# taekkii/deblurgs

Measured on AMD Instinct MI355X. Metric: subframe-renders/sec (fwd+bwd), 1M Gaussians, K=15, 1080p, 1/2/4/8 GPU, higher is better.
Workload: dtype f32; 1 GPU; metric: P=1000000 Gaussians, 1920x1080, K=15 subframes fused, curve_order=3, SH degree 2 (M=9); one blurry view per GPU per step; eager_preferred_steps=279, dropped_steps=0, retried_steps=0, tile_cull=True, depth_output=False, ranks_in_process_group=1

## Files before the change

### deblurgs_amd/build.py

```python
import glob
import hashlib
import json
import os
import subprocess
import sys
from concurrent.futures import ThreadPoolExecutor

HERE = os.path.dirname(os.path.abspath(__file__))
CSRC = os.path.join(HERE, "csrc")
OBJ = os.path.join(CSRC, "obj")
LIB = os.path.join(HERE, "libdgs_hip.so")
ARCH = "gfx950"
SOURCES = {
    "preprocess.hip": ["-ffp-contract=off"],
    "binning.hip": ["-ffp-contract=off"],
    "composite.hip": ["-fno-slp-vectorize"],
    "geometry_bwd.hip": [],
    "pose.hip": [],
    "knn.hip": [],
    "optim.hip": ["-ffp-contract=off"],
    "api.hip": [],
    "loss.hip": [],
    "metrics.hip": ["-ffp-contract=off"],
    "frames.hip": ["-ffp-contract=off"],
    "report.hip": ["-ffp-contract=off"],
    "lpips.hip": ["-ffp-contract=off"],
    "listprof.hip": [],
    "register.hip": [],
    "scene.hip": ["-ffp-contract=off"],
    "png.hip": [],
}
COMMON = ["-O3", "-fPIC", "-std=c++17", f"--offload-arch={ARCH}", "-fhip-fp32-correctly-rounded-divide-sqrt",
          "-Wall", "-Wno-unused-function"]


def _hipcc():
    for c in (os.environ.get("HIPCC"), "/opt/rocm/bin/hipcc", "hipcc"):
        if c and (os.path.isabs(c) and os.path.exists(c) or not os.path.isabs(c)):
            return c
    return "hipcc"


def _stale(target, deps):
    if not os.path.exists(target):
        return True
    t = os.path.getmtime(target)
    return any(os.path.getmtime(d) > t for d in deps)


HEADER = os.path.join(HERE, "..", "include", "dgs_hip.h")


def _sha(*chunks):
    h = hashlib.sha256()
    for c in chunks:
        h.update(c if isinstance(c, bytes) else c.encode())
        h.update(b"\0")
    return h.hexdigest()


def _read(path):
    with open(path, "rb") as f:
        return f.read()


def flag_table():
    return json.dumps({"common": COMMON, "sources": SOURCES, "arch": ARCH}, sort_keys=True)


def build_id(csrc=CSRC, header=HEADER):
    parts = []
    for f in sorted(glob.glob(os.path.join(csrc, "*.hip")) + glob.glob(os.path.join(csrc, "*.h"))):
        parts += [os.path.basename(f), _read(f)]
    parts += ["dgs_hip.h", _read(header), flag_table()]
    return _sha(*parts)


def _object_stamp(src, extra, headers, bid):
    return _sha(_read(src), *[_read(h) for h in headers], json.dumps(COMMON + extra), bid if src.endswith("api.hip") else "")


def _stamp_matches(path, want):
    try:
        with open(path) as f:
            return f.read().strip() == want
    except OSError:
        return False


SAN_LIB = os.path.join(HERE, "libdgs_hip_san.so")
SAN_OBJ = os.path.join(CSRC, "obj_san")
SAN_FLAGS = ["-O1", "-g", "-fno-omit-frame-pointer", "-fsanitize=address,undefined", "-fno-gpu-sanitize", "-shared-libsan",
             "-fno-sanitize-recover=undefined"]


def asan_runtime():
    r = subprocess.run([_hipcc(), "-print-file-name=libclang_rt.asan-x86_64.so"], capture_output=True, text=True)
    path = r.stdout.strip()
    if os.path.isabs(path) and os.path.exists(path):
        return path
    import glob
    hits = glob.glob("/opt/rocm/lib/llvm/lib/clang/*/lib/linux/libclang_rt.asan-x86_64.so")
    return hits[0] if hits else None


def build_sanitized(force=False, verbose=False):
    os.makedirs(SAN_OBJ, exist_ok=True)
    headers = [os.path.join(CSRC, "dgs_common.h"), os.path.join(HERE, "..", "include", "dgs_hip.h")]
    hipcc = _hipcc()
    common = [f for f in COMMON if f != "-O3"] + SAN_FLAGS
    jobs, objs = [], []
    for src, extra in SOURCES.items():
        s = os.path.join(CSRC, src)
        o = os.path.join(SAN_OBJ, src.replace(".hip", ".o"))
        objs.append(o)
        if force or _stale(o, [s] + headers):
            define = [f'-DDGS_BUILD_ID="{build_id()}"'] if src == "api.hip" else []
            jobs.append([hipcc] + common + extra + define + ["-c", s, "-o", o])

    def run(cmd):
        if verbose:
            print(" ".join(cmd), flush=True)
        r = subprocess.run(cmd, capture_output=True, text=True)
        if r.returncode != 0:
            raise RuntimeError("hipcc failed:\n" + " ".join(cmd) + "\n" + r.stdout + r.stderr)
        return r

    with ThreadPoolExecutor(max_workers=4) as ex:
        list(ex.map(run, jobs))
    if force or jobs or _stale(SAN_LIB, objs):
        run([hipcc, "-shared", "-fPIC", f"--offload-arch={ARCH}", "-fsanitize=address,undefined", "-shared-libsan",
             "-o", SAN_LIB] + objs)
    return SAN_LIB


def build(force=False, verbose=False):
    os.makedirs(OBJ, exist_ok=True)
    headers = [os.path.join(CSRC, "dgs_common.h"), HEADER]
    hipcc = _hipcc()
    bid = build_id()
    jobs = []
    objs = []
    stamps = []
    for src, extra in SOURCES.items():
        s = os.path.join(CSRC, src)
        o = os.path.join(OBJ, src.replace(".hip", ".o"))
        objs.append(o)
        want = _object_stamp(s, extra, headers, bid)
        if force or not os.path.exists(o) or not _stamp_matches(o + ".stamp", want):
            define = [f'-DDGS_BUILD_ID="{bid}"'] if src == "api.hip" else []
            jobs.append([hipcc] + COMMON + extra + define + ["-c", s, "-o", o])
            stamps.append((o + ".stamp", want))

    def run(cmd):
        if verbose:
            print(" ".join(cmd), flush=True)
        r = subprocess.run(cmd, capture_output=True, text=True)
        if r.returncode != 0:
            raise RuntimeError("hipcc failed:\n" + " ".join(cmd) + "\n" + r.stdout + r.stderr)
        return r

    with ThreadPoolExecutor(max_workers=4) as ex:
        list(ex.map(run, jobs))
    for path, want in stamps:
        with open(path, "w") as f:
            f.write(want + "\n")
    if force or jobs or not os.path.exists(LIB) or not _stamp_matches(LIB + ".stamp", bid):
        run([hipcc, "-shared", "-fPIC", f"--offload-arch={ARCH}", "-o", LIB] + objs)
        with open(LIB + ".stamp", "w") as f:
            f.write(bid + "\n")
    return LIB


if __name__ == "__main__":
    if "--sanitize" in sys.argv:
        print(build_sanitized(force="--force" in sys.argv, verbose=True))
    else:
        print(build(force="--force" in sys.argv, verbose=True))
```

### deblurgs_amd/csrc/api.hip

```cpp
#include <stdio.h>
#include <string.h>

#include <mutex>
#include <new>

#include "dgs_common.h"

namespace {

thread_local char g_err[512] = "";

int fail(int code, const char* fmt, const char* a = "") {
  snprintf(g_err, sizeof(g_err), fmt, a);
  return code;
}
int fail_hip(hipError_t e, const char* where) {
  snprintf(g_err, sizeof(g_err), "%s: %s", where, hipGetErrorString(e));
  return DGS_E_HIP;
}

constexpr size_t ALIGN = 256;
size_t up(size_t x) { return (x + ALIGN - 1) / ALIGN * ALIGN; }

int sort_bits_for(int W, int H, int K) {
// ... 53 lines not shown

int check_problem(const DgsProblem* p, bool need_opacity = true) {
  if (p == nullptr) return fail(DGS_E_ARG, "null DgsProblem");
  if (p->P < 0 || p->W <= 0 || p->H <= 0) return fail(DGS_E_ARG, "bad P/W/H");
  if (p->W > 4095 * DGS_TILE || p->H > 4095 * DGS_TILE) return fail(DGS_E_ARG, "W / H above 65520 pixels");
  if (p->K < 1 || p->K > DGS_MAX_K) return fail(DGS_E_ARG, "K must be in [1, DGS_MAX_K]");
  if (p->D < 0 || p->D > 3) return fail(DGS_E_ARG, "SH degree must be 0..3");
  if (p->forward_only != 0 && p->forward_only != 1) return fail(DGS_E_ARG, "forward_only must be 0 or 1");
  if (p->P == 0) return DGS_OK;
  if (p->means3D == nullptr || (need_opacity && p->opacities == nullptr))
    return fail(DGS_E_ARG, "means3D / opacities are null");
  if ((p->shs == nullptr) == (p->colors_precomp == nullptr))
    return fail(DGS_E_ARG, "Please provide excatly one of either SHs or precomputed colors!");
  if (((p->scales == nullptr || p->rotations == nullptr) && p->cov3D_precomp == nullptr) ||
      ((p->scales != nullptr || p->rotations != nullptr) && p->cov3D_precomp != nullptr))
    return fail(DGS_E_ARG, "Please provide exactly one of either scale/rotation pair or precomputed 3D covariance!");
  if (p->shs != nullptr && p->M < (p->D + 1) * (p->D + 1)) return fail(DGS_E_ARG, "M < (D+1)^2");
  if (p->raw_params != 0 && p->raw_params != 1 && p->raw_params != 3)
    return fail(DGS_E_ARG, "raw_params must be 0, 1 or 3 (1 | isotropic scale)");
  if (p->raw_params) {
    if (p->shs == nullptr || p->scales == nullptr || p->rotations == nullptr)
      return fail(DGS_E_ARG, "raw_params needs shs (dc), scales and rotations");
    if (p->M > 1 && p->shs_rest == nullptr) return fail(DGS_E_ARG, "raw_params with M > 1 needs shs_rest");
  } else if (p->shs_rest != nullptr) {
    return fail(DGS_E_ARG, "shs_rest is only meaningful with raw_params");
  }
  if (p->viewmatrix == nullptr || p->projmatrix == nullptr || p->campos == nullptr || p->bg == nullptr)
    return fail(DGS_E_ARG, "viewmatrix / projmatrix / campos / bg are null");
  if ((uint64_t)p->K * (uint64_t)p->P >= (1ull << 32)) return fail(DGS_E_ARG, "K*P must be < 2^32");
  return DGS_OK;
}

DgsView make_view(const DgsProblem* p, const DgsLayout& L) {
  DgsView v;
  v.P = p->P; v.D = p->D; v.M = p->M; v.W = p->W; v.H = p->H; v.K = p->K;
  v.gx = (p->W + DGS_TILE - 1) / DGS_TILE;
  v.gy = (p->H + DGS_TILE - 1) / DGS_TILE;
  v.T = v.gx * v.gy;
  v.tanfovx = p->tanfovx; v.tanfovy = p->tanfovy;
  v.focal_y = p->H / (2.0f * p->tanfovy);
  v.focal_x = p->W / (2.0f * p->tanfovx);
  v.scale_modifier = p->scale_modifier;
  v.z_far = p->z_far;
  v.use_sigmoid = p->use_sigmoid; v.prefiltered = p->prefiltered;
  v.tile_cull = p->tile_cull != 0;
  v.raw_params = (p->raw_params & 1) != 0;
  v.iso_scale = (p->raw_params & 2) != 0;
  v.pack_g_shift = v.tile_cull ? L.pack_g_shift : 0;
  v.pack_tile_shift = v.tile_cull ? L.pack_tile_shift : 0;
  v.scale_lb = p->scale_lb;
  return v;
}

void carve(const DgsProblem* p, const DgsLayout& L, DgsCarve* c) {
  char* g = reinterpret_cast<char*>(p->geom_state);
  char* im = reinterpret_cast<char*>(p->image_state);
  char* b = reinterpret_cast<char*>(p->binning_state);
  c->rows = reinterpret_cast<DgsRow*>(g + L.geom_rows);
  c->cov3D = p->forward_only ? nullptr : reinterpret_cast<float*>(g + L.cov3D);
  c->pre_sigmoid = p->forward_only ? nullptr : reinterpret_cast<float*>(g + L.pre_sigmoid);
  c->tiles_touched = reinterpret_cast<uint32_t*>(g + L.tiles_touched);
  c->point_offsets = reinterpret_cast<uint32_t*>(g + L.point_offsets);
  c->scan_tmp = reinterpret_cast<uint32_t*>(g + L.scan_tmp);
  c->num_rendered = reinterpret_cast<uint32_t*>(g + L.num_rendered);
  c->gsort_keys = reinterpret_cast<uint32_t*>(g + L.gsort_keys);
  c->gsort_keys_alt = reinterpret_cast<uint32_t*>(g + L.gsort_keys_alt);
  c->gsort_vals = reinterpret_cast<uint32_t*>(g + L.gsort_vals);
  c->gsort_vals_alt = reinterpret_cast<uint32_t*>(g + L.gsort_vals_alt);
  c->tt_sorted = reinterpret_cast<uint32_t*>(g + L.tt_sorted);
  c->offs_sorted = reinterpret_cast<uint32_t*>(g + L.offs_sorted);
  c->tt_tight = reinterpret_cast<uint32_t*>(g + L.tt_tight);
  c->offs_tight = reinterpret_cast<uint32_t*>(g + L.offs_tight);
  c->gsort_tmp = reinterpret_cast<uint32_t*>(g + L.gsort_tmp);
  c->cull_rec = reinterpret_cast<uint4*>(g + L.cull_rec);
  c->cull_cnt = reinterpret_cast<uint32_t*>(g + L.cull_cnt);
  c->final_T = p->forward_only ? nullptr : reinterpret_cast<float*>(im + L.final_T);
  c->n_contrib = p->forward_only ? nullptr : reinterpret_cast<uint32_t*>(im + L.n_contrib);
  c->ranges = reinterpret_cast<uint2*>(im + L.ranges);
  c->keys_sorted = b ? reinterpret_cast<uint64_t*>(b + L.keys_sorted) : nullptr;
  c->point_list = b ? reinterpret_cast<uint32_t*>(b + L.point_list) : nullptr;
  c->keys_unsorted = b ? reinterpret_cast<uint64_t*>(b + L.keys_unsorted) : nullptr;
  c->vals_unsorted = b ? reinterpret_cast<uint32_t*>(b + L.vals_unsorted) : nullptr;
  c->sort_tmp = b ? reinterpret_cast<uint32_t*>(b + L.sort_tmp) : nullptr;
}

struct ScratchLayout {
  size_t sums, partials, total;
};
ScratchLayout scratch_layout(uint64_t R, int P, int K) {
  const size_t sums = up((size_t)R * DGS_CONTRIB_F * 4);
  const size_t partials = sums + up((size_t)K * (size_t)P * DGS_SUMS_F * 4);
  return {sums, partials, partials + up((size_t)dgs_geometry_bwd_blocks(P) * (size_t)K * 24 * 8) + ALIGN};
}

struct Call {
  DgsLayout L;
  DgsCarve c;
  DgsView v;
  float* contrib = nullptr;
  float* sums = nullptr;
  double* partials = nullptr;
};
enum { NEED_IMAGE = 1, NEED_BINNING = 2 };
int prepare(const DgsProblem* p, uint64_t R, int need, const DgsBackwardIO* io, Call* k) {
  k->L = make_layout(p->P, p->W, p->H, p->K, R, p->wide_records != 0, p->forward_only != 0);
  if (p->geom_state == nullptr || p->geom_bytes < k->L.geom_total) return fail(DGS_E_CAPACITY, "geom_state too small");
  if ((need & NEED_IMAGE) && (p->image_state == nullptr || p->image_bytes < k->L.image_total))
    return fail(DGS_E_CAPACITY, "image_state too small");
  if ((need & NEED_BINNING) && R > 0 && (p->binning_state == nullptr || p->binning_bytes < k->L.binning_total))
    return fail(DGS_E_CAPACITY, "binning_state too small");
  carve(p, k->L, &k->c);
  k->v = make_view(p, k->L);
  if (io != nullptr) {
    const ScratchLayout sl = scratch_layout(R, p->P, p->K);
    if (io->scratch == nullptr || io->scratch_bytes < sl.total) return fail(DGS_E_CAPACITY, "backward scratch too small");
    char* base = reinterpret_cast<char*>(io->scratch);
    k->contrib = reinterpret_cast<float*>(base);
    k->sums = reinterpret_cast<float*>(base + sl.sums);
    k->partials = reinterpret_cast<double*>(base + sl.partials);
  }
  return DGS_OK;
}

constexpr int PROF_MAX = 16384;
struct Prof {
  bool on = false;
  int n = 0;
  hipEvent_t* beg = nullptr;
  hipEvent_t* end = nullptr;
  int* stage = nullptr;
  int created = 0;
};
}

struct DgsContext {
  std::mutex mu;
  DgsContextOptions opt;
  bool side_ready = false;
  int side_device = -1;
  hipStream_t s2 = nullptr;
  hipEvent_t done[DGS_MAX_BWD_PARTS] = {}, join = nullptr;
  Prof prof;
};

namespace {

int prof_begin(DgsContext* ctx, int stage, hipStream_t s) {
  if (ctx == nullptr || !ctx->prof.on) return -1;
  Prof& pr = ctx->prof;
  std::lock_guard<std::mutex> lk(ctx->mu);
  if (pr.n >= PROF_MAX) return -1;
  const int i = pr.n++;
  if (i >= pr.created) {
    (void)hipEventCreate(&pr.beg[i]);
    (void)hipEventCreate(&pr.end[i]);
    pr.created = i + 1;
  }
  pr.stage[i] = stage;
  (void)hipEventRecord(pr.beg[i], s);
  return i;
}
void prof_end(DgsContext* ctx, int i, hipStream_t s) {
  if (i >= 0) (void)hipEventRecord(ctx->prof.end[i], s);
}

struct StageTimer {
  DgsContext* ctx;
  int id;
  hipStream_t s;
  StageTimer(DgsContext* c, int stage, hipStream_t st) : ctx(c), id(prof_begin(c, stage, st)), s(st) {}
  ~StageTimer() { prof_end(ctx, id, s); }
};

#define DGS_STAGE(stage_id, where, expr)                                   \
  do {                                                                      \
    hipError_t e__;                                                         \
    {                                                                       \
      StageTimer tm__(p->context, stage_id, s);                                         \
      e__ = (expr);                                                         \
    }                                                                       \
    if (e__ != hipSuccess) return fail_hip(e__, where);                     \
    if (p->debug) {                                                         \
      e__ = hipStreamSynchronize(s);                                        \
      if (e__ != hipSuccess) return fail_hip(e__, where " (debug sync)");   \
    }                                                                       \
  } while (0)

}

int dgs_fail_arg(const char* msg) { return fail(DGS_E_ARG, "%s", msg); }
int dgs_fail_hip(hipError_t e, const char* where) { return fail_hip(e, where); }

extern "C" {

// ... 552 lines not shown
```

### deblurgs_amd/csrc/composite.hip

```cpp
#include <type_traits>

#include "dgs_common.h"

namespace {

typedef float v2f __attribute__((ext_vector_type(2)));

constexpr int CW = 4;

struct TileCtx {
  int k, tx, ty;
  uint32_t r0, r1;
};

__device__ __forceinline__ uint32_t xcd_remap(uint32_t b, uint32_t per_xcd) { return (b & 7u) * per_xcd + (b >> 3); }

__device__ __forceinline__ bool load_tile_ctx(const DgsView& v, const uint2* __restrict__ ranges, uint32_t per_xcd,
                                              TileCtx& t) {
  const uint32_t logical = xcd_remap(blockIdx.x, per_xcd);
  const uint32_t gw = logical * CW + (uint32_t)__builtin_amdgcn_readfirstlane((int)(threadIdx.x >> 6));
  const uint32_t KT = (uint32_t)v.K * (uint32_t)v.T;
  if (gw >= KT) return false;
  t.k = (int)(gw / (uint32_t)v.T);
  const uint32_t tile = gw - (uint32_t)t.k * (uint32_t)v.T;
  t.ty = (int)(tile / (uint32_t)v.gx);
  t.tx = (int)(tile - (uint32_t)t.ty * (uint32_t)v.gx);
  const uint2 r = ranges[gw];
  t.r0 = r.x;
  t.r1 = r.y;
  return true;
}

#ifndef DGS_LOG2_CONIC
#define DGS_LOG2_CONIC 0
#endif
#if DGS_LOG2_CONIC
constexpr float K_LOG2E = -1.4426950408889634f;
constexpr float K_HALF_LOG2E = -0.7213475204444817f;
#else
constexpr float K_LOG2E = -1.0f;
constexpr float K_HALF_LOG2E = -0.5f;
#endif
__device__ __forceinline__ float dgs_power2(float A, float B, float C, float dx, float dy) {
  const float u = fmaf(B, dy, A * dx);
#if DGS_LOG2_CONIC
  return fmaf(C * dy, dy, dx * u);
#else
  return fmaf(C * dy, dy, dx * u) * 1.4426950408889634f;
#endif
}

#ifndef DGS_EXACT_POWER
#define DGS_EXACT_POWER 0
#endif
#ifndef DGS_DIV_REFINE
#define DGS_DIV_REFINE 0
#endif
#if DGS_EXACT_POWER
__device__ __forceinline__ float dgs_power_ref(float a, float b, float c, float dx, float dy) {
  const float t0 = __fmul_rn(__fmul_rn(a, dx), dx), t1 = __fmul_rn(__fmul_rn(c, dy), dy);
  const float t2 = __fmul_rn(__fmul_rn(b, dx), dy);
  return __fsub_rn(__fmul_rn(-0.5f, __fadd_rn(t0, t1)), t2);
}
#endif

__device__ __forceinline__ float dgs_min_raw(float c, float x) {
  float r;
  asm("v_min_f32 %0, %1, %2" : "=v"(r) : "v"(c), "v"(x));
  return r;
}

#ifndef DGS_TIMELINE
#define DGS_TIMELINE 0
#endif
#if DGS_TIMELINE
__device__ unsigned long long* g_timeline = nullptr;
#endif

using CullGauss = DgsCull;
#define make_cull dgs_make_cull
#define cull_hit dgs_cull_hit

template <bool WITHDEPTH, bool KEEP, bool CHK = false>
__global__ void __launch_bounds__(64 * CW)
composite_fwd_kernel(DgsView v, uint32_t per_xcd, const uint2* __restrict__ ranges,
                     const uint32_t* __restrict__ point_list, const uint64_t* __restrict__ keys,
                     const DgsRow* __restrict__ rows,
                     const float* __restrict__ bg, float* __restrict__ final_T, uint32_t* __restrict__ n_contrib,
                     float* __restrict__ out_color, float* __restrict__ out_depth, uint32_t* __restrict__ checksum = nullptr) {
  __shared__ float4 s_row[CW][64 * 3];
  TileCtx t;
  if (!load_tile_ctx(v, ranges, per_xcd, t)) return;
  const int lane = dgs_lane(), w = __builtin_amdgcn_readfirstlane((int)(threadIdx.x >> 6));
  const int lx = lane & 7, ly = lane >> 3;
  const int px0 = t.tx * DGS_TILE + lx, py0 = t.ty * DGS_TILE + ly;
  const float pxf0 = (float)px0, pxf1 = (float)(px0 + 8), pyf0 = (float)py0, pyf1 = (float)(py0 + 8);
  const float qx0 = (float)(t.tx * DGS_TILE), qy0 = (float)(t.ty * DGS_TILE);

  float T[4], C0[4], C1[4], C2[4], Dd[4];
  uint32_t last[4], chk[4];
#pragma unroll
  for (int q = 0; q < 4; q++) {
    C0[q] = C1[q] = C2[q] = Dd[q] = 0.0f;
    last[q] = 0;
    chk[q] = 0;
    const int px = px0 + (q & 1) * 8, py = py0 + (q >> 1) * 8;
    T[q] = (px < v.W && py < v.H) ? 1.0f : -1.0f;
  }
  const DgsRow* krows = rows + (size_t)t.k * v.P;
  const uint32_t n = t.r1 - t.r0;
  uint64_t alive[4];
#pragma unroll
  for (int q = 0; q < 4; q++) alive[q] = __ballot(T[q] > 0.0f);

  for (uint32_t base = 0; base < n; base += 64) {
    if ((alive[0] | alive[1] | alive[2] | alive[3]) == 0) break;
    const bool has = base + lane < n;
    float4 A = make_float4(0, 0, 0, 0), B = A, Cc = A;
    if (has) {
      const uint32_t g = v.pack_tile_shift > 0
                             ? (uint32_t)(keys[t.r0 + base + lane] >> v.pack_g_shift) &
                                   ((1u << (v.pack_tile_shift - v.pack_g_shift)) - 1u)
                             : point_list[t.r0 + base + lane];
      const float4* rp = reinterpret_cast<const float4*>(krows + g);
      A = rp[0];
      B = rp[1];
      Cc = rp[2];
    }
    const CullGauss cg = make_cull(A.z, A.w, B.x, B.y);
    const uint64_t pdm = __ballot(!cg.always);
    uint64_t m[4];
#pragma unroll
    for (int q = 0; q < 4; q++) {
      const float ex = A.x - (qx0 + (float)((q & 1) * 8)), ey = A.y - (qy0 + (float)((q >> 1) * 8));
      const bool hit = has && cull_hit(cg, ex - 7.0f, ex, ey - 7.0f, ey);
      const uint64_t bh = __ballot(hit);
      m[q] = alive[q] ? bh : 0ull;
    }
#if DGS_EXACT_POWER
    s_row[w][3 * lane] = make_float4(A.x, A.y, A.z, A.w);
    s_row[w][3 * lane + 1] = make_float4(B.x, B.y, B.z, B.w);
#else
    s_row[w][3 * lane] = make_float4(A.x, A.y, A.z * K_HALF_LOG2E, A.w * K_LOG2E);
    s_row[w][3 * lane + 1] = make_float4(B.x * K_HALF_LOG2E, B.y, B.z, B.w);
#endif
    s_row[w][3 * lane + 2] = make_float4(Cc.x, Cc.y, 0.0f, 0.0f);
    __builtin_amdgcn_fence(__ATOMIC_RELEASE, "wavefront");
    __builtin_amdgcn_wave_barrier();
    __builtin_amdgcn_fence(__ATOMIC_ACQUIRE, "wavefront");

    const uint64_t mu_all = m[0] | m[1] | m[2] | m[3];
    auto run_batch = [&](auto checkc) {
    constexpr bool CHECK = decltype(checkc)::value;
    uint64_t mu = mu_all;
    while (mu) {
      const int j = __builtin_ctzll(mu);
      mu &= mu - 1;
      const float4* rowj = &s_row[w][3 * j];
      const float4 a = rowj[0];
      const float4 b = rowj[1];
      const float2 c = *reinterpret_cast<const float2*>(rowj + 2);
      uint32_t posv = base + (uint32_t)j + 1u;
      asm volatile("" : "+v"(posv));
#pragma unroll
      for (int q = 0; q < 4; q++) {
        if ((m[q] >> j) & 1ull) {
          const float dx = a.x - ((q & 1) ? pxf1 : pxf0);
          const float dy = a.y - ((q >> 1) ? pyf1 : pyf0);
#if DGS_EXACT_POWER
          const float power = dgs_power_ref(a.z, a.w, b.x, dx, dy);
          const float alpha_raw = fminf(0.99f, b.y * __builtin_amdgcn_exp2f(power * 1.4426950408889634f));
          const bool ok = (power <= 0.0f) && (alpha_raw >= 1.0f / 255.0f);
#else
          const float power = dgs_power2(a.z, a.w, b.x, dx, dy);
          const float alpha_raw = fminf(0.99f, b.y * __builtin_amdgcn_exp2f(power));
          const bool ok = (!CHECK || power <= 0.0f) && (alpha_raw >= 1.0f / 255.0f);
#endif
          const float alpha = ok ? alpha_raw : 0.0f;
          const float test_T = T[q] * (1.0f - alpha);
          const bool stop = test_T < 0.0001f;
          const float wgt = stop ? 0.0f : alpha * T[q];
          C0[q] += b.z * wgt;
          C1[q] += b.w * wgt;
          C2[q] += c.x * wgt;
          if (WITHDEPTH) Dd[q] += c.y * wgt;
          T[q] = stop ? -fabsf(T[q]) : test_T;
          if (KEEP) last[q] = (ok && !stop) ? posv : last[q];
          if (CHK) chk[q] += (ok && !stop) ? posv * 2654435761u : 0u;
        }
      }
    }
    };
    if ((~pdm & mu_all) == 0ull)
      run_batch(std::false_type{});
    else
      run_batch(std::true_type{});
#pragma unroll
    for (int q = 0; q < 4; q++) alive[q] = __ballot(T[q] > 0.0f);
    __builtin_amdgcn_wave_barrier();
  }

  const float bg0 = bg[0], bg1 = bg[1], bg2 = bg[2];
  const size_t N = (size_t)v.W * v.H;
#pragma unroll
  for (int q = 0; q < 4; q++) {
    const int px = px0 + (q & 1) * 8, py = py0 + (q >> 1) * 8;
    if (px < v.W && py < v.H) {
      const size_t pix = (size_t)py * v.W + px;
      const float Tf = fabsf(T[q]);
      if (KEEP) {
        final_T[(size_t)t.k * N + pix] = Tf;
        n_contrib[(size_t)t.k * N + pix] = last[q];
      }
      float* oc = out_color + (size_t)t.k * 3 * N;
      oc[pix] = C0[q] + Tf * bg0;
      oc[N + pix] = C1[q] + Tf * bg1;
      oc[2 * N + pix] = C2[q] + Tf * bg2;
      if (WITHDEPTH) out_depth[(size_t)t.k * N + pix] = Dd[q] + Tf * v.z_far;
      if (CHK) checksum[(size_t)t.k * N + pix] = chk[q];
    }
  }
}

template <bool TIGHT, bool HASDEPTH, bool POSE = false>
__global__ void __launch_bounds__(64 * CW)
composite_bwd_kernel(DgsView v, uint32_t per_xcd, const uint2* __restrict__ ranges,
                     const uint32_t* __restrict__ point_list, const uint64_t* __restrict__ keys,
                     const DgsRow* __restrict__ rows,
                     const float* __restrict__ bg, const float* __restrict__ final_T,
                     const uint32_t* __restrict__ n_contrib, const float* __restrict__ dL_dpix,
                     const float* __restrict__ dL_ddepth, const uint32_t* __restrict__ dup_off,
                     float* __restrict__ contrib) {
  __shared__ float4 s_row[CW][64 * 3];
  __shared__ __attribute__((aligned(16))) float s_part[CW][10][68];
  TileCtx t;
  if (!load_tile_ctx(v, ranges, per_xcd, t)) return;
#if DGS_TIMELINE
  const unsigned long long t_begin = wall_clock64();
#endif
  const int lane = dgs_lane(), w = __builtin_amdgcn_readfirstlane((int)(threadIdx.x >> 6));
  const int lx = lane & 7, ly = lane >> 3;
  const int px0 = t.tx * DGS_TILE + lx, py0 = t.ty * DGS_TILE + ly;
  const float pxf0 = (float)px0, pxf1 = (float)(px0 + 8), pyf0 = (float)py0, pyf1 = (float)(py0 + 8);
  const float qx0 = (float)(t.tx * DGS_TILE), qy0 = (float)(t.ty * DGS_TILE);
  const size_t N = (size_t)v.W * v.H;
  const float bg0 = bg[0], bg1 = bg[1], bg2 = bg[2];
  const int rrow = lane >> 2, rq = lane & 3;
  const bool rlane = rrow < (POSE ? (HASDEPTH ? 6 : 5) : (HASDEPTH ? 10 : 9));
  float* const contrib_lane = contrib + (rrow < 10 ? rrow : 0);
  static_assert(sizeof(float) * 68 == 272, "the store offsets below are multiples of one s_part row");
  const uint32_t part_base = (uint32_t)__builtin_amdgcn_readfirstlane((int)(uint32_t)(size_t)(&s_part[w][0][0]));
  

  float T[4];
  v2f gA[4], gB[4];
  float accg[4];
  uint32_t last[4];
  uint32_t maxc = 0;
#pragma unroll
  for (int q = 0; q < 4; q++) {
    const int px = px0 + (q & 1) * 8, py = py0 + (q >> 1) * 8;
    const bool inside = (px < v.W && py < v.H);
    const size_t pix = (size_t)py * v.W + px;
    const float Tfin = inside ? final_T[(size_t)t.k * N + pix] : 0.0f;
    T[q] = Tfin;
    last[q] = inside ? n_contrib[(size_t)t.k * N + pix] : 0u;
    const float* gp = dL_dpix + (size_t)t.k * 3 * N;
    const float g0 = inside ? gp[pix] : 0.0f;
    const float g1 = inside ? gp[N + pix] : 0.0f;
    const float g2 = inside ? gp[2 * N + pix] : 0.0f;
    const float gd = (inside && dL_ddepth != nullptr) ? dL_ddepth[(size_t)t.k * N + pix] : 0.0f;
    gA[q] = (v2f){g0, g1};
    gB[q] = (v2f){g2, gd};
    accg[q] = bg0 * g0 + bg1 * g1 + bg2 * g2 + v.z_far * gd;
    maxc = max(maxc, last[q]);
  }
  uint32_t maxq[4];
#pragma unroll
  for (int q = 0; q < 4; q++) {
    uint32_t mq = last[q];
#pragma unroll
    for (int d = 32; d >= 1; d >>= 1) mq = max(mq, (uint32_t)__shfl_xor((int)mq, d, 64));
    maxq[q] = __builtin_amdgcn_readfirstlane(mq);
  }
  maxc = max(max(maxq[0], maxq[1]), max(maxq[2], maxq[3]));

  const DgsRow* krows = rows + (size_t)t.k * v.P;
  const uint32_t n = t.r1 - t.r0;
  const uint32_t nbatch = (n + 63) / 64;
  for (uint32_t bi = nbatch; bi-- > 0;) {
    const uint32_t base = bi * 64;
    const bool has = base + lane < n;
    float4 A = make_float4(0, 0, 0, 0), B = A, Cc = A;
    uint32_t u = 0;
    if (has) {
      uint32_t g;
      if (TIGHT && v.pack_tile_shift > 0) {
        const uint64_t key = keys[t.r0 + base + lane];
        g = (uint32_t)(key >> v.pack_g_shift) & ((1u << (v.pack_tile_shift - v.pack_g_shift)) - 1u);
        u = (uint32_t)(key & ((1ull << v.pack_g_shift) - 1ull));
      } else {
        g = point_list[t.r0 + base + lane];
        if (TIGHT) u = reinterpret_cast<const uint32_t*>(keys)[2 * (size_t)(t.r0 + base + lane)];
      }
      const float4* rp = reinterpret_cast<const float4*>(krows + g);
      A = rp[0];
      B = rp[1];
      Cc = rp[2];
      if (!TIGHT) {
        int minx, miny, maxx, maxy;
        dgs_get_rect(A.x, A.y, __float_as_int(Cc.w), v.gx, v.gy, minx, miny, maxx, maxy);
        u = dup_off[(size_t)t.k * v.P + g] + (uint32_t)((t.ty - miny) * (maxx - minx) + (t.tx - minx));
      }
    }
    uint64_t m[4] = {0, 0, 0, 0};
    uint64_t pdm = 0;
    if (base < maxc) {
      const CullGauss cg = make_cull(A.z, A.w, B.x, B.y);
      pdm = __ballot(!cg.always);
#pragma unroll
      for (int q = 0; q < 4; q++) {
        const float ex = A.x - (qx0 + (float)((q & 1) * 8)), ey = A.y - (qy0 + (float)((q >> 1) * 8));
        const bool hit = has && (base + lane < maxq[q]) && cull_hit(cg, ex - 7.0f, ex, ey - 7.0f, ey);
        m[q] = __ballot(hit);
      }
#if DGS_EXACT_POWER
      s_row[w][3 * lane] = make_float4(A.x, A.y, A.z, A.w);
      s_row[w][3 * lane + 1] = make_float4(B.x, B.y, B.z, B.w);
#else
      s_row[w][3 * lane] = make_float4(A.x, A.y, A.z * K_HALF_LOG2E, A.w * K_LOG2E);
      s_row[w][3 * lane + 1] = make_float4(B.x * K_HALF_LOG2E, B.y, B.z, B.w);
#endif
      s_row[w][3 * lane + 2] = HASDEPTH ? make_float4(Cc.x, Cc.y, __uint_as_float(u), 0.0f)
                                        : make_float4(Cc.x, __uint_as_float(u), 0.0f, 0.0f);
    }
    const float4 z4 = make_float4(0, 0, 0, 0);
    if (has && (((m[0] | m[1] | m[2] | m[3]) >> lane) & 1ull) == 0ull) {
      float4* dst = reinterpret_cast<float4*>(contrib + (size_t)u * DGS_CONTRIB_F);
      dst[0] = z4;
      dst[1] = z4;
      if (!POSE) dst[2] = z4;
    }
    __builtin_amdgcn_fence(__ATOMIC_RELEASE, "wavefront");
    __builtin_amdgcn_wave_barrier();
    __builtin_amdgcn_fence(__ATOMIC_ACQUIRE, "wavefront");

    const uint64_t mu_all = m[0] | m[1] | m[2] | m[3];
    auto run_batch = [&](auto checkc) {
    constexpr bool CHECK = decltype(checkc)::value;
    uint64_t mu = mu_all;
    while (mu) {
      const int j = 63 - __builtin_clzll(mu);
      mu &= ~(1ull << j);
      const float4* rowj = &s_row[w][3 * j];
      const float4 a = rowj[0];
      const float4 b = rowj[1];
      float2 c;
      uint32_t uj;
      if (HASDEPTH) {
        const float4 c4 = rowj[2];
        c = make_float2(c4.x, c4.y);
        uj = __float_as_uint(c4.z);
      } else {
        const float2 c2 = *reinterpret_cast<const float2*>(rowj + 2);
        c = make_float2(c2.x, 0.0f);
        uj = __float_as_uint(c2.y);
      }
      const uint32_t pos = base + (uint32_t)j;
      float S_w = 0, S_wx = 0, S_wy = 0, S_xx = 0, S_xy = 0, S_yy = 0;
      v2f sA = {0.0f, 0.0f}, sB = {0.0f, 0.0f};
      const v2f colA = {b.z, b.w}, colB = {c.x, c.y};
      auto pass = [&](auto qc) __attribute__((always_inline)) {
          constexpr int q = decltype(qc)::value;
          const float dx = a.x - ((q & 1) ? pxf1 : pxf0);
          const float dy = a.y - ((q >> 1) ? pyf1 : pyf0);
#if DGS_EXACT_POWER
          const float power = dgs_power_ref(a.z, a.w, b.x, dx, dy);
          const float au_any = b.y * __builtin_amdgcn_exp2f(power * 1.4426950408889634f);
          const bool ok = (pos < last[q]) && (power <= 0.0f) && (au_any >= 1.0f / 255.0f);
#else
          const float power = dgs_power2(a.z, a.w, b.x, dx, dy);
          const float au_any = b.y * __builtin_amdgcn_exp2f(power);
          const bool ok = (pos < last[q]) && (!CHECK || power <= 0.0f) && (au_any >= 1.0f / 255.0f);
#endif
          const float au = ok ? au_any : 0.0f;
          const float alpha = dgs_min_raw(0.99f, au);
#if DGS_EXACT_POWER
          T[q] = T[q] / (1.0f - alpha);
#elif DGS_DIV_REFINE
          const float one_m = 1.0f - alpha;
          const float inv1ma = __builtin_amdgcn_rcpf(one_m);
          const float q0 = T[q] * inv1ma;
          T[q] = fmaf(fmaf(-one_m, q0, T[q]), inv1ma, q0);
#else
          const float inv1ma = __builtin_amdgcn_rcpf(1.0f - alpha);
          T[q] = T[q] * inv1ma;
#endif
          const float dchannel_dcolor = alpha * T[q];
          float cg = fmaf(colB.x, gB[q].x, fmaf(colA.y, gA[q].y, colA.x * gA[q].x));
          if (HASDEPTH) cg = fmaf(colB.y, gB[q].y, cg);
          const float behind = cg - accg[q];
          accg[q] = fmaf(alpha, behind, accg[q]);
          const float wgt = au * (behind * T[q]);
          const float wx = wgt * dx, wy = wgt * dy;
          if (!POSE) {
            sA.x = fmaf(gA[q].x, dchannel_dcolor, sA.x);
            sA.y = fmaf(gA[q].y, dchannel_dcolor, sA.y);
            sB.x = fmaf(gB[q].x, dchannel_dcolor, sB.x);
          }
          if (HASDEPTH) sB.y = fmaf(gB[q].y, dchannel_dcolor, sB.y);
          if (!POSE) S_w += wgt;
          S_wx += wx;
          S_wy += wy;
          S_xx = fmaf(wx, dx, S_xx);
          S_xy = fmaf(wx, dy, S_xy);
          S_yy = fmaf(wy, dy, S_yy);
      };
      using I0 = std::integral_constant<int, 0>;
      using I1 = std::integral_constant<int, 1>;
      using I2 = std::integral_constant<int, 2>;
      using I3 = std::integral_constant<int, 3>;
      if ((m[0] >> j) & 1ull) pass(I0{});
      if ((m[1] >> j) & 1ull) pass(I1{});
      if ((m[2] >> j) & 1ull) pass(I2{});
      if ((m[3] >> j) & 1ull) pass(I3{});
      {
        if (POSE && HASDEPTH)
          asm volatile(
              "s_mov_b32 m0, %6\n\ts_nop 0\n\t"
              "ds_write_addtid_b32 %0 offset:0\n\tds_write_addtid_b32 %1 offset:272\n\t"
              "ds_write_addtid_b32 %2 offset:544\n\tds_write_addtid_b32 %3 offset:816\n\t"
              "ds_write_addtid_b32 %4 offset:1088\n\tds_write_addtid_b32 %5 offset:1360"
              :: "v"(S_wx), "v"(S_wy), "v"(S_xx), "v"(S_xy), "v"(S_yy), "v"(sB.y), "s"(part_base) : "m0", "memory");
        else if (POSE)
          asm volatile(
              "s_mov_b32 m0, %5\n\ts_nop 0\n\t"
              "ds_write_addtid_b32 %0 offset:0\n\tds_write_addtid_b32 %1 offset:272\n\t"
              "ds_write_addtid_b32 %2 offset:544\n\tds_write_addtid_b32 %3 offset:816\n\t"
              "ds_write_addtid_b32 %4 offset:1088"
              :: "v"(S_wx), "v"(S_wy), "v"(S_xx), "v"(S_xy), "v"(S_yy), "s"(part_base) : "m0", "memory");
        else if (HASDEPTH)
          asm volatile(
              "s_mov_b32 m0, %10\n\ts_nop 0\n\t"
              "ds_write_addtid_b32 %0 offset:0\n\tds_write_addtid_b32 %1 offset:272\n\t"
              "ds_write_addtid_b32 %2 offset:544\n\tds_write_addtid_b32 %3 offset:816\n\t"
              "ds_write_addtid_b32 %4 offset:1088\n\tds_write_addtid_b32 %5 offset:1360\n\t"
              "ds_write_addtid_b32 %6 offset:1632\n\tds_write_addtid_b32 %7 offset:1904\n\t"
              "ds_write_addtid_b32 %8 offset:2176\n\tds_write_addtid_b32 %9 offset:2448"
              :: "v"(S_wx), "v"(S_wy), "v"(S_xx), "v"(S_xy), "v"(S_yy), "v"(S_w), "v"(sA.x), "v"(sA.y), "v"(sB.x),
                 "v"(sB.y), "s"(part_base) : "m0", "memory");
        else
          asm volatile(
              "s_mov_b32 m0, %9\n\ts_nop 0\n\t"
              "ds_write_addtid_b32 %0 offset:0\n\tds_write_addtid_b32 %1 offset:272\n\t"
              "ds_write_addtid_b32 %2 offset:544\n\tds_write_addtid_b32 %3 offset:816\n\t"
              "ds_write_addtid_b32 %4 offset:1088\n\tds_write_addtid_b32 %5 offset:1360\n\t"
              "ds_write_addtid_b32 %6 offset:1632\n\tds_write_addtid_b32 %7 offset:1904\n\t"
              "ds_write_addtid_b32 %8 offset:2176"
              :: "v"(S_wx), "v"(S_wy), "v"(S_xx), "v"(S_xy), "v"(S_yy), "v"(S_w), "v"(sA.x), "v"(sA.y), "v"(sB.x),
                 "s"(part_base) : "m0", "memory");
        __builtin_amdgcn_fence(__ATOMIC_RELEASE, "wavefront");
        __builtin_amdgcn_wave_barrier();
        __builtin_amdgcn_fence(__ATOMIC_ACQUIRE, "wavefront");
        float tot = 0.0f;
        if (rlane) {
          const float4* pr = reinterpret_cast<const float4*>(&s_part[w][rrow][16 * rq]);
          const float4 x0 = pr[0], x1 = pr[1], x2 = pr[2], x3 = pr[3];
          tot = (((x0.x + x0.y) + (x0.z + x0.w)) + ((x1.x + x1.y) + (x1.z + x1.w))) +
                (((x2.x + x2.y) + (x2.z + x2.w)) + ((x3.x + x3.y) + (x3.z + x3.w)));
        }
        tot = dgs_quad_sum(tot);
        asm volatile("" : "+v"(tot));
        {
          if (rrow < (POSE ? 8 : 10) && rq == 0) contrib_lane[(size_t)uj * DGS_CONTRIB_F] = tot;
        }
        __builtin_amdgcn_wave_barrier();
      }
    }
    };
    if ((~pdm & mu_all) == 0ull)
      run_batch(std::false_type{});
    else
      run_batch(std::true_type{});
    __builtin_amdgcn_fence(__ATOMIC_RELEASE, "wavefront");
    __builtin_amdgcn_wave_barrier();
    __builtin_amdgcn_fence(__ATOMIC_ACQUIRE, "wavefront");
    __builtin_amdgcn_wave_barrier();
  }
#if DGS_TIMELINE
  if (lane == 0 && g_timeline != nullptr) {
    const size_t gw = (size_t)t.k * v.T + (size_t)t.ty * v.gx + t.tx;
    g_timeline[3 * gw] = t_begin;
    g_timeline[3 * gw + 1] = wall_clock64();
    g_timeline[3 * gw + 2] = ((unsigned long long)(blockIdx.x * CW + w) << 16) |
                             ((unsigned long long)__builtin_amdgcn_s_getreg((3 << 11) | 20) << 8) |
                             (unsigned long long)(blockIdx.x & 7u);
  }
#endif
}

}

#if DGS_TIMELINE
extern "C" int dgs_debug_set_timeline(void* buffer) {
  unsigned long long* p = reinterpret_cast<unsigned long long*>(buffer);
  return hipMemcpyToSymbol(HIP_SYMBOL(g_timeline), &p, sizeof(p)) == hipSuccess ? 0 : -3;
}
#endif

static uint32_t per_xcd_blocks(const DgsView& v) {
  const uint64_t KT = (uint64_t)v.K * v.T;
  const uint64_t nblk = (KT + CW - 1) / CW;
  return (uint32_t)((nblk + 7) / 8);
}

hipError_t dgs_launch_composite_fwd(const DgsView& v, const DgsCarve& c, const float* bg, float* out_color,
                                    float* out_depth, hipStream_t s, uint32_t* checksum) {
  const uint32_t per = per_xcd_blocks(v);
  if (per == 0) return hipSuccess;
#define DGS_CFWD(WD, KP)                                                                                                  \
  hipLaunchKernelGGL((composite_fwd_kernel<WD, KP>), dim3(per * 8), dim3(64 * CW), 0, s, v, per, c.ranges, c.point_list, \
                     c.keys_sorted, c.rows, bg, c.final_T, c.n_contrib, out_color, out_depth)
  const bool keep = c.final_T != nullptr && c.n_contrib != nullptr;
  if (checksum != nullptr) {
    if (out_depth == nullptr || !keep) return hipErrorInvalidValue;
    hipLaunchKernelGGL((composite_fwd_kernel<true, true, true>), dim3(per * 8), dim3(64 * CW), 0, s, v, per, c.ranges,
                       c.point_list, c.keys_sorted, c.rows, bg, c.final_T, c.n_contrib, out_color, out_depth, checksum);
    return hipGetLastError();
  }
  if (out_depth != nullptr) {
    if (keep) DGS_CFWD(true, true); else DGS_CFWD(true, false);
  } else {
    if (keep) DGS_CFWD(false, true); else DGS_CFWD(false, false);
  }
#undef DGS_CFWD
  return hipGetLastError();
}

hipError_t dgs_launch_composite_bwd(const DgsView& v_all, const DgsCarve& c, const float* bg, const float* dL_dpix,
                                    const float* dL_ddepth, float* contrib, hipStream_t s, int k0, int k1, bool pose) {
  if (k1 < 0) { k0 = 0; k1 = v_all.K; }
  DgsView v = v_all;
  v.K = k1 - k0;
  const size_t N = (size_t)v.W * v.H;
  const uint32_t per = per_xcd_blocks(v);
  if (per == 0) return hipSuccess;
  const uint2* ranges = c.ranges + (size_t)k0 * v.T;
  const DgsRow* rows = c.rows + (size_t)k0 * v.P;
  const float* final_T = c.final_T + (size_t)k0 * N;
  const uint32_t* n_contrib = c.n_contrib + (size_t)k0 * N;
  dL_dpix += (size_t)k0 * 3 * N;
  if (dL_ddepth != nullptr) dL_ddepth += (size_t)k0 * N;
#define DGS_CBWD(TI, HD, ...)                                                                                       \
  hipLaunchKernelGGL((composite_bwd_kernel<TI, HD, ##__VA_ARGS__>), dim3(per * 8), dim3(64 * CW), 0, s, v, per, ranges, c.point_list, \
                     c.keys_sorted, rows, bg, final_T, n_contrib, dL_dpix, dL_ddepth, c.point_offsets, contrib)
  if (pose) {
    if (v.tile_cull) {
      if (dL_ddepth != nullptr) DGS_CBWD(true, true, true); else DGS_CBWD(true, false, true);
    } else {
      if (dL_ddepth != nullptr) DGS_CBWD(false, true, true); else DGS_CBWD(false, false, true);
    }
  } else if (v.tile_cull) {
    if (dL_ddepth != nullptr) DGS_CBWD(true, true); else DGS_CBWD(true, false);
  } else {
    if (dL_ddepth != nullptr) DGS_CBWD(false, true); else DGS_CBWD(false, false);
  }
#undef DGS_CBWD
  return hipGetLastError();
}
```

### deblurgs_amd/csrc/dgs_common.h

```cpp
#pragma once
#include <hip/hip_runtime.h>
#include <stdint.h>

#include "../../include/dgs_hip.h"

#define DGS_TILE 16
#define DGS_DEPTH_KEY_BASE 0x3E4CCCCDu
#define DGS_ROW_F 12
#define DGS_CONTRIB_F 12
#define DGS_SUMS_F 16
#define DGS_WAVE 64

struct __attribute__((aligned(16))) DgsRow {
  float x, y;
  float cx, cy, cz, op;
  float r, g, b, depth;
  uint32_t dup_offset;
  int32_t radius;
};
static_assert(sizeof(DgsRow) == 4 * DGS_ROW_F, "row must be 48 bytes");

struct DgsCarve {
  DgsRow* rows;
  float* cov3D;
  float* pre_sigmoid;
  uint32_t* tiles_touched;
  uint32_t* point_offsets;
  uint32_t* scan_tmp;
  uint32_t* num_rendered;
  uint32_t* gsort_keys;
  uint32_t* gsort_keys_alt;
  uint32_t* gsort_vals;
  uint32_t* gsort_vals_alt;
  uint32_t* tt_sorted;
  uint32_t* offs_sorted;
  uint32_t* tt_tight;
  uint32_t* offs_tight;
  uint32_t* gsort_tmp;
  uint4* cull_rec;
  uint32_t* cull_cnt;
  float* final_T;
  uint32_t* n_contrib;
  uint2* ranges;
  uint64_t* keys_sorted;
  uint32_t* point_list;
  uint64_t* keys_unsorted;
  uint32_t* vals_unsorted;
  uint32_t* sort_tmp;
};

static inline uint32_t dgs_higher_msb64(uint64_t n) {
  uint32_t b = 0;
  while (b < 64 && (n >> b) != 0) b++;
  return b;
}
static inline uint32_t dgs_higher_msb(uint32_t n) {
  uint32_t msb = sizeof(n) * 4;
  uint32_t step = msb;
  while (step > 1) {
    step /= 2;
    if (n >> msb)
      msb += step;
    else
      msb -= step;
  }
  if (n >> msb) msb++;
  return msb;
}

__device__ __forceinline__ void dgs_get_rect(float px, float py, int max_radius, int gx, int gy, int& minx,
                                             int& miny, int& maxx, int& maxy) {
  minx = min(gx, max(0, (int)((px - max_radius) / DGS_TILE)));
  miny = min(gy, max(0, (int)((py - max_radius) / DGS_TILE)));
  maxx = min(gx, max(0, (int)((px + max_radius + DGS_TILE - 1) / DGS_TILE)));
  maxy = min(gy, max(0, (int)((py + max_radius + DGS_TILE - 1) / DGS_TILE)));
}

template <int CTRL, int ROW_MASK>
__device__ __forceinline__ float dgs_dpp(float v) {
  return __int_as_float(__builtin_amdgcn_update_dpp(0, __float_as_int(v), CTRL, ROW_MASK, 0xf, false));
}

__device__ __forceinline__ float dgs_wave_sum63(float v) {
  v += dgs_dpp<0xB1, 0xf>(v);
  v += dgs_dpp<0x4E, 0xf>(v);
  v += dgs_dpp<0x141, 0xf>(v);
  v += dgs_dpp<0x140, 0xf>(v);
  v += dgs_dpp<0x142, 0xa>(v);
  v += dgs_dpp<0x143, 0xc>(v);
  return v;
}

__device__ __forceinline__ int dgs_lane() { return (int)(threadIdx.x & 63); }

__device__ __forceinline__ float dgs_quad_sum(float v) {
  v += dgs_dpp<0xB1, 0xf>(v);
  v += dgs_dpp<0x4E, 0xf>(v);
  return v;
}
__device__ __forceinline__ float dgs_row_sum(float v) {
  v += dgs_dpp<0xB1, 0xf>(v);
  v += dgs_dpp<0x4E, 0xf>(v);
  v += dgs_dpp<0x141, 0xf>(v);
  v += dgs_dpp<0x140, 0xf>(v);
  return v;
}

__device__ __forceinline__ float dgs_sgn(float x) { return (x > 0.0f) ? 1.0f : ((x < 0.0f) ? -1.0f : 0.0f); }

constexpr double DGS_TOTALS_FX = 16777216.0;
template <typename T>
__device__ __forceinline__ bool dgs_totals_publish(T a, T c, float* __restrict__ work, unsigned long long& t0,
                                                   unsigned long long& t1, bool& bad) {
  unsigned long long* acc = reinterpret_cast<unsigned long long*>(work + 2);
  unsigned int* flag = reinterpret_cast<unsigned int*>(work + 7);
  const bool fin = __builtin_isfinite(a) && __builtin_isfinite(c) && a < (T)5.0e11 && c < (T)5.0e11;
  if (!fin) {
    atomicOr(flag, 1u);
  } else {
    const unsigned long long ia = (unsigned long long)__double2ll_rn((double)a * DGS_TOTALS_FX);
    const unsigned long long ic = (unsigned long long)__double2ll_rn((double)c * DGS_TOTALS_FX);
    const unsigned long long oa = atomicAdd(&acc[0], ia), oc = atomicAdd(&acc[1], ic);
    if (oa + ia < oa || oc + ic < oc) atomicOr(flag, 1u);
  }
  __threadfence();
  const unsigned int ticket = atomicAdd(reinterpret_cast<unsigned int*>(work + 6), 1u);
  if (ticket != gridDim.x - 1) return false;
  __threadfence();
  t0 = atomicAdd(&acc[0], 0ull);
  t1 = atomicAdd(&acc[1], 0ull);
  bad = atomicOr(flag, 0u) != 0u;
// ... 107 lines not shown
```

Measured before the change: 1417 subframe-renders/sec.

## Reuse forward-pass per-batch hit masks in composite backward instead of recomputing culls

```diff
diff --git a/deblurgs_amd/build.py b/deblurgs_amd/build.py
--- a/deblurgs_amd/build.py
+++ b/deblurgs_amd/build.py
@@ -106,7 +106,7 @@
 
 def build_sanitized(force=False, verbose=False):
     os.makedirs(SAN_OBJ, exist_ok=True)
-    headers = [os.path.join(CSRC, "dgs_common.h"), os.path.join(HERE, "..", "include", "dgs_hip.h")]
+    headers = sorted(glob.glob(os.path.join(CSRC, "*.h"))) + [os.path.join(HERE, "..", "include", "dgs_hip.h")]
     hipcc = _hipcc()
     common = [f for f in COMMON if f != "-O3"] + SAN_FLAGS
     jobs, objs = [], []
@@ -136,7 +136,7 @@
 
 def build(force=False, verbose=False):
     os.makedirs(OBJ, exist_ok=True)
-    headers = [os.path.join(CSRC, "dgs_common.h"), HEADER]
+    headers = sorted(glob.glob(os.path.join(CSRC, "*.h"))) + [HEADER]
     hipcc = _hipcc()
     bid = build_id()
     jobs = []
diff --git a/deblurgs_amd/csrc/api.hip b/deblurgs_amd/csrc/api.hip
--- a/deblurgs_amd/csrc/api.hip
+++ b/deblurgs_amd/csrc/api.hip
@@ -159,6 +159,9 @@
   c->keys_unsorted = b ? reinterpret_cast<uint64_t*>(b + L.keys_unsorted) : nullptr;
   c->vals_unsorted = b ? reinterpret_cast<uint32_t*>(b + L.vals_unsorted) : nullptr;
   c->sort_tmp = b ? reinterpret_cast<uint32_t*>(b + L.sort_tmp) : nullptr;
+  c->after_sort = b ? reinterpret_cast<unsigned char*>(b + L.keys_unsorted) : nullptr;
+  c->after_sort_bytes = b ? L.binning_total - L.keys_unsorted : 0;
+  c->list_capacity = 0;
 }
 
 struct ScratchLayout {
@@ -187,6 +190,11 @@
   if ((need & NEED_BINNING) && R > 0 && (p->binning_state == nullptr || p->binning_bytes < k->L.binning_total))
     return fail(DGS_E_CAPACITY, "binning_state too small");
   carve(p, k->L, &k->c);
+  if (p->binning_state == nullptr || p->binning_bytes < k->L.binning_total) {
+    k->c.after_sort = nullptr;
+    k->c.after_sort_bytes = 0;
+  }
+  k->c.list_capacity = R;
   k->v = make_view(p, k->L);
   if (io != nullptr) {
     const ScratchLayout sl = scratch_layout(R, p->P, p->K);
diff --git a/deblurgs_amd/csrc/composite.hip b/deblurgs_amd/csrc/composite.hip
--- a/deblurgs_amd/csrc/composite.hip
+++ b/deblurgs_amd/csrc/composite.hip
@@ -1,6 +1,11 @@
 #include <type_traits>
 
 #include "dgs_common.h"
+#include "pass_records.h"
+
+#ifndef DGS_BWD_FWD_MASKS
+#define DGS_BWD_FWD_MASKS 1
+#endif
 
 namespace {
 
@@ -11,6 +16,7 @@
 struct TileCtx {
   int k, tx, ty;
   uint32_t r0, r1;
+  uint32_t gw;
 };
 
 __device__ __forceinline__ uint32_t xcd_remap(uint32_t b, uint32_t per_xcd) { return (b & 7u) * per_xcd + (b >> 3); }
@@ -28,6 +34,7 @@
   const uint2 r = ranges[gw];
   t.r0 = r.x;
   t.r1 = r.y;
+  t.gw = gw;
   return true;
 }
 
@@ -75,6 +82,13 @@
 #endif
 #if DGS_TIMELINE
 __device__ unsigned long long* g_timeline = nullptr;
+#endif
+
+#ifndef DGS_PASSCOUNT
+#define DGS_PASSCOUNT 0
+#endif
+#if DGS_PASSCOUNT
+__device__ unsigned long long g_passcount[8];
 #endif
 
 using CullGauss = DgsCull;
@@ -87,7 +101,8 @@
                      const uint32_t* __restrict__ point_list, const uint64_t* __restrict__ keys,
                      const DgsRow* __restrict__ rows,
                      const float* __restrict__ bg, float* __restrict__ final_T, uint32_t* __restrict__ n_contrib,
-                     float* __restrict__ out_color, float* __restrict__ out_depth, uint32_t* __restrict__ checksum = nullptr) {
+                     float* __restrict__ out_color, float* __restrict__ out_depth, uint4* __restrict__ pass_rec,
+                     uint32_t n_rec, uint32_t* __restrict__ checksum = nullptr) {
   __shared__ float4 s_row[CW][64 * 3];
   TileCtx t;
   if (!load_tile_ctx(v, ranges, per_xcd, t)) return;
@@ -113,6 +128,9 @@
 #pragma unroll
   for (int q = 0; q < 4; q++) alive[q] = __ballot(T[q] > 0.0f);
 
+#if DGS_PASSCOUNT
+  unsigned long long pc_adm = 0, pc_con = 0, pc_ent = 0, pc_cent = 0, pc_bat = 0;
+#endif
   for (uint32_t base = 0; base < n; base += 64) {
     if ((alive[0] | alive[1] | alive[2] | alive[3]) == 0) break;
     const bool has = base + lane < n;
@@ -149,6 +167,15 @@
     __builtin_amdgcn_wave_barrier();
     __builtin_amdgcn_fence(__ATOMIC_ACQUIRE, "wavefront");
 
+#if DGS_BWD_FWD_MASKS
+    if (KEEP && pass_rec != nullptr) {
+      const uint32_t rec = dgs_pass_record_index(t.r0, t.gw, base >> 6);
+      if (rec < n_rec && lane == 0) {
+        pass_rec[2 * (size_t)rec] = make_uint4((uint32_t)m[0], (uint32_t)(m[0] >> 32), (uint32_t)m[1], (uint32_t)(m[1] >> 32));
+        pass_rec[2 * (size_t)rec + 1] = make_uint4((uint32_t)m[2], (uint32_t)(m[2] >> 32), (uint32_t)m[3], (uint32_t)(m[3] >> 32));
+      }
+    }
+#endif
     const uint64_t mu_all = m[0] | m[1] | m[2] | m[3];
     auto run_batch = [&](auto checkc) {
     constexpr bool CHECK = decltype(checkc)::value;
@@ -162,6 +189,10 @@
       const float2 c = *reinterpret_cast<const float2*>(rowj + 2);
       uint32_t posv = base + (uint32_t)j + 1u;
       asm volatile("" : "+v"(posv));
+#if DGS_PASSCOUNT
+      bool pc_any = false;
+      pc_ent++;
+#endif
 #pragma unroll
       for (int q = 0; q < 4; q++) {
         if ((m[q] >> j) & 1ull) {
@@ -187,10 +218,20 @@
           T[q] = stop ? -fabsf(T[q]) : test_T;
           if (KEEP) last[q] = (ok && !stop) ? posv : last[q];
           if (CHK) chk[q] += (ok && !stop) ? posv * 2654435761u : 0u;
+#if DGS_PASSCOUNT
+          pc_adm++;
+          if (__ballot(ok && !stop) != 0ull) { pc_con++; pc_any = true; }
+#endif
         }
       }
+#if DGS_PASSCOUNT
+      if (pc_any) pc_cent++;
+#endif
     }
     };
+#if DGS_PASSCOUNT
+    pc_bat++;
+#endif
     if ((~pdm & mu_all) == 0ull)
       run_batch(std::false_type{});
     else
@@ -200,6 +241,15 @@
     __builtin_amdgcn_wave_barrier();
   }
 
+#if DGS_PASSCOUNT
+  if (lane == 0) {
+    atomicAdd(&g_passcount[0], pc_adm);
+    atomicAdd(&g_passcount[1], pc_con);
+    atomicAdd(&g_passcount[2], pc_ent);
+    atomicAdd(&g_passcount[3], pc_cent);
+    atomicAdd(&g_passcount[4], pc_bat);
+  }
+#endif
   const float bg0 = bg[0], bg1 = bg[1], bg2 = bg[2];
   const size_t N = (size_t)v.W * v.H;
 #pragma unroll
@@ -222,7 +272,7 @@
   }
 }
 
-template <bool TIGHT, bool HASDEPTH, bool POSE = false>
+template <bool TIGHT, bool HASDEPTH, bool POSE, bool FM>
 __global__ void __launch_bounds__(64 * CW)
 composite_bwd_kernel(DgsView v, uint32_t per_xcd, const uint2* __restrict__ ranges,
                      const uint32_t* __restrict__ point_list, const uint64_t* __restrict__ keys,
@@ -230,7 +280,7 @@
                      const float* __restrict__ bg, const float* __restrict__ final_T,
                      const uint32_t* __restrict__ n_contrib, const float* __restrict__ dL_dpix,
                      const float* __restrict__ dL_ddepth, const uint32_t* __restrict__ dup_off,
-                     float* __restrict__ contrib) {
+                     float* __restrict__ contrib, const uint4* __restrict__ pass_rec, uint32_t n_rec, uint32_t rec_gw0) {
   __shared__ float4 s_row[CW][64 * 3];
   __shared__ __attribute__((aligned(16))) float s_part[CW][10][68];
   TileCtx t;
@@ -318,11 +368,28 @@
     if (base < maxc) {
       const CullGauss cg = make_cull(A.z, A.w, B.x, B.y);
       pdm = __ballot(!cg.always);
-#pragma unroll
-      for (int q = 0; q < 4; q++) {
-        const float ex = A.x - (qx0 + (float)((q & 1) * 8)), ey = A.y - (qy0 + (float)((q >> 1) * 8));
-        const bool hit = has && (base + lane < maxq[q]) && cull_hit(cg, ex - 7.0f, ex, ey - 7.0f, ey);
-        m[q] = __ballot(hit);
+      if (FM) {
+        const uint32_t rec = (uint32_t)__builtin_amdgcn_readfirstlane(
+            (int)dgs_pass_record_index(t.r0, rec_gw0 + t.gw, bi));
+        uint4 lo = make_uint4(0u, 0u, 0u, 0u), hi = lo;
+        if (rec < n_rec) {
+          lo = pass_rec[2 * (size_t)rec];
+          hi = pass_rec[2 * (size_t)rec + 1];
+        }
+        const uint64_t rm[4] = {((uint64_t)lo.y << 32) | lo.x, ((uint64_t)lo.w << 32) | lo.z,
+                                ((uint64_t)hi.y << 32) | hi.x, ((uint64_t)hi.w << 32) | hi.z};
+#pragma unroll
+        for (int q = 0; q < 4; q++) {
+          const uint64_t below = maxq[q] <= base ? 0ull : (maxq[q] - base >= 64u ? ~0ull : (1ull << (maxq[q] - base)) - 1ull);
+          m[q] = rm[q] & below;
+        }
+      } else {
+#pragma unroll
+        for (int q = 0; q < 4; q++) {
+          const float ex = A.x - (qx0 + (float)((q & 1) * 8)), ey = A.y - (qy0 + (float)((q >> 1) * 8));
+          const bool hit = has && (base + lane < maxq[q]) && cull_hit(cg, ex - 7.0f, ex, ey - 7.0f, ey);
+          m[q] = __ballot(hit);
+        }
       }
 #if DGS_EXACT_POWER
       s_row[w][3 * lane] = make_float4(A.x, A.y, A.z, A.w);
@@ -346,6 +413,14 @@
     __builtin_amdgcn_fence(__ATOMIC_ACQUIRE, "wavefront");
 
     const uint64_t mu_all = m[0] | m[1] | m[2] | m[3];
+#if DGS_PASSCOUNT
+    if (lane == 0) {
+      atomicAdd(&g_passcount[5], (unsigned long long)(__builtin_popcountll(m[0]) + __builtin_popcountll(m[1]) +
+                                                      __builtin_popcountll(m[2]) + __builtin_popcountll(m[3])));
+      atomicAdd(&g_passcount[6], (unsigned long long)__builtin_popcountll(mu_all));
+      if (base < maxc) atomicAdd(&g_passcount[7], 1ull);
+    }
+#endif
     auto run_batch = [&](auto checkc) {
     constexpr bool CHECK = decltype(checkc)::value;
     uint64_t mu = mu_all;
@@ -501,6 +576,15 @@
 
 }
 
+#if DGS_PASSCOUNT
+extern "C" int dgs_debug_passcount(unsigned long long* out8) {
+  unsigned long long z[8] = {0, 0, 0, 0, 0, 0, 0, 0};
+  if (hipDeviceSynchronize() != hipSuccess) return -3;
+  if (out8 != nullptr && hipMemcpyFromSymbol(out8, HIP_SYMBOL(g_passcount), sizeof(z)) != hipSuccess) return -3;
+  return hipMemcpyToSymbol(HIP_SYMBOL(g_passcount), z, sizeof(z)) == hipSuccess ? 0 : -3;
+}
+#endif
+
 #if DGS_TIMELINE
 extern "C" int dgs_debug_set_timeline(void* buffer) {
   unsigned long long* p = reinterpret_cast<unsigned long long*>(buffer);
@@ -514,18 +598,37 @@
   return (uint32_t)((nblk + 7) / 8);
 }
 
+static uint4* pass_records(const DgsView& v_all, const DgsCarve& c, uint32_t* n_rec) {
+  *n_rec = 0;
+#if DGS_BWD_FWD_MASKS
+  const uint64_t n = dgs_pass_record_count(c.list_capacity, (uint64_t)v_all.K * (uint64_t)v_all.T);
+  if (c.after_sort == nullptr || c.list_capacity == 0 || n >= (1ull << 32) ||
+      n * DGS_PASS_RECORD_BYTES > (uint64_t)c.after_sort_bytes)
+    return nullptr;
+  *n_rec = (uint32_t)n;
+  return reinterpret_cast<uint4*>(c.after_sort);
+#else
+  (void)v_all;
+  (void)c;
+  return nullptr;
+#endif
+}
+
 hipError_t dgs_launch_composite_fwd(const DgsView& v, const DgsCarve& c, const float* bg, float* out_color,
                                     float* out_depth, hipStream_t s, uint32_t* checksum) {
   const uint32_t per = per_xcd_blocks(v);
   if (per == 0) return hipSuccess;
+  uint32_t n_rec = 0;
+  uint4* const rec = pass_records(v, c, &n_rec);
 #define DGS_CFWD(WD, KP)                                                                                                  \
   hipLaunchKernelGGL((composite_fwd_kernel<WD, KP>), dim3(per * 8), dim3(64 * CW), 0, s, v, per, c.ranges, c.point_list, \
-                     c.keys_sorted, c.rows, bg, c.final_T, c.n_contrib, out_color, out_depth)
+                     c.keys_sorted, c.rows, bg, c.final_T, c.n_contrib, out_color, out_depth, rec, n_rec)
   const bool keep = c.final_T != nullptr && c.n_contrib != nullptr;
   if (checksum != nullptr) {
     if (out_depth == nullptr || !keep) return hipErrorInvalidValue;
     hipLaunchKernelGGL((composite_fwd_kernel<true, true, true>), dim3(per * 8), dim3(64 * CW), 0, s, v, per, c.ranges,
-                       c.point_list, c.keys_sorted, c.rows, bg, c.final_T, c.n_contrib, out_color, out_depth, checksum);
+                       c.point_list, c.keys_sorted, c.rows, bg, c.final_T, c.n_contrib, out_color, out_depth, rec, n_rec,
+                       checksum);
     return hipGetLastError();
   }
   if (out_depth != nullptr) {
@@ -551,9 +654,19 @@
   const uint32_t* n_contrib = c.n_contrib + (size_t)k0 * N;
   dL_dpix += (size_t)k0 * 3 * N;
   if (dL_ddepth != nullptr) dL_ddepth += (size_t)k0 * N;
-#define DGS_CBWD(TI, HD, ...)                                                                                       \
-  hipLaunchKernelGGL((composite_bwd_kernel<TI, HD, ##__VA_ARGS__>), dim3(per * 8), dim3(64 * CW), 0, s, v, per, ranges, c.point_list, \
-                     c.keys_sorted, rows, bg, final_T, n_contrib, dL_dpix, dL_ddepth, c.point_offsets, contrib)
+  uint32_t n_rec = 0;
+  const uint4* const rec = pass_records(v_all, c, &n_rec);
+  const uint32_t rec_gw0 = (uint32_t)k0 * (uint32_t)v.T;
+#define DGS_CBWD_FM(TI, HD, PO, FM)                                                                                            \
+  hipLaunchKernelGGL((composite_bwd_kernel<TI, HD, PO, FM>), dim3(per * 8), dim3(64 * CW), 0, s, v, per, ranges, c.point_list, \
+                     c.keys_sorted, rows, bg, final_T, n_contrib, dL_dpix, dL_ddepth, c.point_offsets, contrib, rec, n_rec,  \
+                     rec_gw0)
+#if DGS_BWD_FWD_MASKS
+#define DGS_CBWD(TI, HD, PO) \
+  do { if (rec != nullptr) DGS_CBWD_FM(TI, HD, PO, true); else DGS_CBWD_FM(TI, HD, PO, false); } while (0)
+#else
+#define DGS_CBWD(TI, HD, PO) DGS_CBWD_FM(TI, HD, PO, false)
+#endif
   if (pose) {
     if (v.tile_cull) {
       if (dL_ddepth != nullptr) DGS_CBWD(true, true, true); else DGS_CBWD(true, false, true);
@@ -561,10 +674,11 @@
       if (dL_ddepth != nullptr) DGS_CBWD(false, true, true); else DGS_CBWD(false, false, true);
     }
   } else if (v.tile_cull) {
-    if (dL_ddepth != nullptr) DGS_CBWD(true, true); else DGS_CBWD(true, false);
+    if (dL_ddepth != nullptr) DGS_CBWD(true, true, false); else DGS_CBWD(true, false, false);
   } else {
-    if (dL_ddepth != nullptr) DGS_CBWD(false, true); else DGS_CBWD(false, false);
+    if (dL_ddepth != nullptr) DGS_CBWD(false, true, false); else DGS_CBWD(false, false, false);
   }
 #undef DGS_CBWD
+#undef DGS_CBWD_FM
   return hipGetLastError();
 }
diff --git a/deblurgs_amd/csrc/dgs_common.h b/deblurgs_amd/csrc/dgs_common.h
--- a/deblurgs_amd/csrc/dgs_common.h
+++ b/deblurgs_amd/csrc/dgs_common.h
@@ -47,6 +47,9 @@
   uint64_t* keys_unsorted;
   uint32_t* vals_unsorted;
   uint32_t* sort_tmp;
+  unsigned char* after_sort;
+  size_t after_sort_bytes;
+  uint64_t list_capacity;
 };
 
 static inline uint32_t dgs_higher_msb64(uint64_t n) {
diff --git a/deblurgs_amd/csrc/pass_records.h b/deblurgs_amd/csrc/pass_records.h
--- /dev/null
+++ b/deblurgs_amd/csrc/pass_records.h
@@ -0,0 +1,16 @@
+#ifndef DGS_PASS_RECORDS_H
+#define DGS_PASS_RECORDS_H
+#include <stdint.h>
+
+#if defined(__HIPCC__) || defined(__CUDACC__)
+#define DGS_PR_FN static __host__ __device__ __forceinline__
+#else
+#define DGS_PR_FN static inline
+#endif
+
+#define DGS_PASS_RECORD_BYTES 32u
+
+DGS_PR_FN uint64_t dgs_pass_record_count(uint64_t R, uint64_t KT) { return (R >> 6) + KT; }
+DGS_PR_FN uint32_t dgs_pass_record_index(uint32_t r0, uint32_t gw, uint32_t bi) { return (r0 >> 6) + gw + bi; }
+
+#endif
```

Result: no change. 1431 subframe-renders/sec (median of 6 runs) (+1.0%).
